# lan496/torch-m3gnet

Measured on AMD Instinct MI355X. Metric: atom-steps/sec (energy+forces) on 10k-atom PBC batch, 1/2/4/8 MI355X, higher is better.
Workload: dtype f32; 1 GPU; single 10000-atom fcc Cu PBC supercell per GPU (10x10x25 cells, a=3.61 A, jitter 0.025 A), r_cut 5 A / 3-body 4 A, default M3GNet (l_max=n_max=3, D=64, 3 blocks), energy+forces+stress; precision=fp32, atoms_per_gpu=10000, edges_per_gpu=420000, triplets_per_gpu=3060000

## Files before the change

torch-m3gnet_amd/csrc/m3g_api.hip:

```cpp
#include <cmath>
#include <cstdarg>
#include <cstdio>
#include <cstdlib>
#include <cstring>

#include "m3g_internal.h"

namespace m3g {

static thread_local char g_err[512] = "";
void set_error(const char* fmt, ...) {
  va_list ap;
  va_start(ap, fmt);
  vsnprintf(g_err, sizeof(g_err), fmt, ap);
  va_end(ap);
}

static inline size_t align_up(size_t x, size_t a = 256) { return (x + a - 1) / a * a; }

static void layout_mlp(MlpW& m, size_t& off) {
  auto take = [&](size_t n) { size_t r = off; off += (n + 63) / 64 * 64; return r; };
  m.w1a_t = take(kDP * 2 * kDP); m.w1b_t = take(kDP * 2 * kDP); m.w1c_t = take(kDP * 2 * kDP);
  m.b1 = take(2 * kDP);
  m.w2d_t = take(kDP * kDP); m.w2g_t = take(kDP * kDP);
// ... 312 lines not shown
    return M3G_OK;
  }
  if (strcmp(name, "save_p1") == 0) {
    plan->save_p1 = value != 0;
    return M3G_OK;
  }
  if (strcmp(name, "save_p2") == 0) {
    plan->save_p2 = value != 0;
    return M3G_OK;
  }
  if (strcmp(name, "rev_kernel") == 0) {
    if (value != 0 && value != 1) { set_error("rev_kernel must be 0 (node-MLP + edge-MLP kernel pair) or 1 (fused)"); return M3G_ERR_VALUE; }
    plan->rev_kernel = value;
    return M3G_OK;
  }
  if (strcmp(name, "small_tiles") == 0) {
    if (value < 0) { set_error("small_tiles must be >= 0"); return M3G_ERR_VALUE; }
    plan->small_tiles = value;
    plan->small_tiles_fwd = value;
    drop_graphs(plan);
    return M3G_OK;
  }
  if (strcmp(name, "small_tiles_fwd") == 0) {
    if (value < 0) { set_error("small_tiles_fwd must be >= 0"); return M3G_ERR_VALUE; }
    plan->small_tiles_fwd = value;
    drop_graphs(plan);
    return M3G_OK;
  }
  if (strcmp(name, "dp1_by_dst") == 0) {
    plan->dp1_by_dst = value != 0;
// ... 228 lines not shown
    M3G_HIP_CHECK(hipStreamWaitEvent(s, plan->ev_fork, 0));
  }
  auto join = [&]() -> int {
    if (via_side) {
      M3G_HIP_CHECK(hipEventRecord(plan->ev_join, s));
      M3G_HIP_CHECK(hipStreamWaitEvent(caller, plan->ev_join, 0));
    }
    return M3G_OK;
  };
  std::vector<unsigned char> key(sizeof(m3g_io) + sizeof(void*) * 2 + sizeof(size_t) + 4 * sizeof(int));
  unsigned char* k = key.data();
  memcpy(k, io, sizeof(m3g_io)); k += sizeof(m3g_io);
  memcpy(k, &workspace, sizeof(void*)); k += sizeof(void*);
  memcpy(k, &s, sizeof(void*)); k += sizeof(void*);
  memcpy(k, &workspace_bytes, sizeof(size_t)); k += sizeof(size_t);
  const int opts[4] = {plan->edge_kernel, plan->rev_kernel + 2 * plan->save_p1 + 4 * plan->save_p2 + 8 * plan->tb_moments + 16 * plan->precision + 64 * plan->readout_f16, plan->stress_mode, plan->overlap};
  memcpy(k, opts, sizeof(opts));
  for (auto& g : plan->graphs)
    if (g.key == key) { M3G_HIP_CHECK(hipGraphLaunch(g.exec, s)); return join(); }
  if (plan->graphs.size() >= 8) drop_graphs(plan);
  m3g_plan::GraphEntry ge;
  ge.key = key;
  M3G_HIP_CHECK(hipStreamBeginCapture(s, hipStreamCaptureModeThreadLocal));
  plan->capturing = true;
  const int rc = m3g_energy_forces(plan, io, workspace, workspace_bytes, (void*)s);
  plan->capturing = false;
  hipError_t e = hipStreamEndCapture(s, &ge.graph);
  if (rc != M3G_OK) { if (ge.graph) (void)hipGraphDestroy(ge.graph); return rc; }
  if (e != hipSuccess || !ge.graph) { set_error("hipStreamEndCapture failed: %s", hipGetErrorString(e)); return M3G_ERR_HIP; }
  e = hipGraphInstantiate(&ge.exec, ge.graph, nullptr, nullptr, 0);
  if (e != hipSuccess) { (void)hipGraphDestroy(ge.graph); set_error("hipGraphInstantiate failed: %s", hipGetErrorString(e)); return M3G_ERR_HIP; }
// ... 270 lines not shown
```

torch-m3gnet_amd/csrc/m3g_edge_common.h:

```cpp
#pragma once
#include <utility>

#include "m3g_device.h"
#include "m3g_internal.h"
#include "m3g_dual_chain.h"
#include "m3g_dual_f32.h"
#include "m3g_mfma_common.h"

namespace m3g {

constexpr int kFwdLdsFloats = 8 * kTbSteps * 64 + 2 * (8 * 4 * 4 * 64 + 2 * (4 * 4 * 4 * 64) + 2 * 4 * 64 + 4 * 64) + 4 * 64;
constexpr int kRevMlpFloats = 8 * 4 * 4 * 64 + 4 * (4 * 4 * 4 * 64) + 2 * 4 * 64 + 4 * 8 * 4 * 64 + 64 * 4;
constexpr int kRevEdgeFloats = kRevMlpFloats + 8 * kTbSteps * 64 + 8 * 4 * 64;
#ifndef M3G_WAVES_FWD
#define M3G_WAVES_FWD 16
#endif
constexpr int kWaves = M3G_WAVES_FWD;
#ifndef M3G_WAVES_FWD_H
#define M3G_WAVES_FWD_H 12
#endif
template <int PREC>
#ifndef M3G_WAVES_FWD_BF
#define M3G_WAVES_FWD_BF 12
#endif
// ... 397 lines not shown
  const float* e2_tile;
  float* de_soa;
  float* dcn;
  int de_is_zero;
  float* dm;
  float* dh;
  float* dp1;
  unsigned long long* stamps;
  float *seg_head, *seg_first;
  const float* p1;
  const float* p2;
  float w_inv;
  float* dp1_scale;
  const int32_t* in_pos;
  int split_tail;
};

__device__ __forceinline__ float sum_lane_quarters(float x) {
  const unsigned u = __builtin_bit_cast(unsigned, x);
  auto r16 = __builtin_amdgcn_permlane16_swap(u, u, false, false);
  const float y = __builtin_bit_cast(float, (unsigned)r16[0]) + __builtin_bit_cast(float, (unsigned)r16[1]);
  const unsigned v = __builtin_bit_cast(unsigned, y);
  auto r32 = __builtin_amdgcn_permlane32_swap(v, v, false, false);
  return __builtin_bit_cast(float, (unsigned)r32[0]) + __builtin_bit_cast(float, (unsigned)r32[1]);
}

__device__ __forceinline__ void store_dh(float* dh, int64_t edge, int64_t E, f32x4 dhv, int qd) {
  static_for<4>([&]<int rr>() { dhv[rr] = sum_lane_quarters(dhv[rr]); });
  if (qd == 0 && edge < E) *(f32x4*)(dh + edge * kRP) = dhv;
}
// ... 31 lines not shown
```

torch-m3gnet_amd/csrc/m3g_edge_rev_f32.hip:

```cpp
#include "m3g_edge_common.h"
#include "m3g_edge_split_rev.h"

namespace m3g {

MfmaRevF32Layout mfma_rev_f32_layout() {
  MfmaRevF32Layout L{};
  int off = 0;
  auto take = [&](int n) { int r = off; off += n; return r; };
  L.tb = take(8 * kTbSteps * 64);
  L.tbT = take(1 * 32 * 64);
  for (int m = 0; m < 2; ++m) {
    L.mlp[m].w2d = take(64 * 64);
    L.mlp[m].w2g = take(64 * 64);
    L.mlp[m].w1cT = take(4 * 32 * 64);
    L.mlp[m].b2 = take(2 * 4 * 64);
    L.mlp[m].wl = take(64 * 4);
    L.mlp[m].wld = take(4 * 64);
  }
  L.adj = take(4 * 64);
  L.adjp = take(64 * 4);
  L.total = off;
  return L;
}

constexpr int kRevF32Floats = 8 * kTbSteps * 64 + 32 * 64 + 2 * (2 * 64 * 64 + 4 * 32 * 64 + 2 * 4 * 64 + 64 * 4 + 4 * 64) + 4 * 64 + 64 * 4;
#ifndef M3G_WAVES_REV_F32
#define M3G_WAVES_REV_F32 8
#endif
constexpr int kWavesRevF32 = M3G_WAVES_REV_F32;

#ifndef M3G_NO_SCHED_FENCE
#define M3G_F32_FENCE() __builtin_amdgcn_sched_barrier(0)
#else
#define M3G_F32_FENCE() ((void)0)
#endif

template <bool NEED_DP1, int MLP, bool SAVED_P2>
__device__ __forceinline__ void mlp_reverse_f32(const float* lds, const MfmaMlpRevF32& L, const RevArgs& a, int64_t edge, int64_t drow, int64_t tile,
                                                int64_t ci, const SegMasks& sk, const f32x4& hv, const f32x4 (&d_upd)[4],
                                                f32x4 (&contrib)[4], f32x4& dhv, int lane, f32x4 (&d2)[8]) {
  const int qd = lane >> 4;
  f32x4 p1[SAVED_P2 ? 1 : 8];
  const float* p1_src = a.p1 + tile * (2 * kP1TileFloats) + MLP * kP1TileFloats + (threadIdx.x & 63) * 4;
  if constexpr (SAVED_P2) {
  } else {
    static_for<8>([&]<int ob>() { p1[ob] = load_tile4(p1_src + ob * 256); });
    bias_step<4, 0>(lds + L.b2, d2, lane);
    bias_step<4, 4>(lds + L.b2 + 4 * 64, d2, lane);
    static_for<2>([&]<int half>() {
      f32x4 hid[4];
      static_for<4>([&]<int ob>() {
        static_for<4>([&]<int r>() {
// ... 40 lines not shown
      const float d_out = du * s_lin, d_s = du * sd * sg;
      dhv[0] += d_s * w[0]; dhv[1] += d_s * w[1]; dhv[2] += d_s * w[2]; dhv[3] += d_s * w[3];
      d2[ob][r] = d_out * sg * (sgd * (1.f + p2d * (1.f - sgd)));
      d2[4 + ob][r] = d_out * sd * sg * (1.f - sg);
    });
#endif
    asm volatile("" : "+v"(dhv[0]), "+v"(dhv[1]), "+v"(dhv[2]), "+v"(dhv[3]));
  });
  zero(contrib);
  M3G_F32_FENCE();
  static_for<2>([&]<int half>() {
    f32x4 dp1[4];
    zero(dp1);
    f32x4 ds1[4];
    if constexpr (SAVED_P2) static_for<4>([&]<int ob>() { ds1[ob] = load_tile4(p1_src + (4 * half + ob) * 256); });
    chain_dual32_t<4, 4 * half, 0>(lds + (half == 0 ? L.w2d : L.w2g), d2, dp1, lane);
    if constexpr (SAVED_P2) static_for<4>([&]<int ob>() { dp1[ob] *= ds1[ob]; });
    else static_for<4>([&]<int ob>() { dp1[ob] *= p1[4 * half + ob]; });
    if (NEED_DP1 && edge < a.E) {
      float* row = a.dp1 + drow * (4 * kDP) + MLP * (2 * kDP) + half * kDP + 4 * qd;
      static_for<4>([&]<int ob>() { *(f32x4*)(row + ob * 16) = dp1[ob]; });
    }
    chain_f32<4, 4, 0, 0, 8, 4 * half>(lds + L.w1cT, dp1, contrib, lane);
    if (NEED_DP1) {
      if (edge >= a.E) zero(dp1);
      seg_scan(dp1, sk);
      seg_store<MLP * 8 + 4 * half>(dp1, sk, a.seg_head, a.seg_first, tile, ci, qd);
    }
    M3G_F32_FENCE();
  });
}

__device__ __forceinline__ void load_p2(const RevArgs& a, int64_t tile, int mlp, f32x4 (&d2)[8]) {
  const float* src = a.p2 + tile * (2 * kP1TileFloats) + mlp * kP1TileFloats + (threadIdx.x & 63) * 4;
  static_for<8>([&]<int ob>() { d2[ob] = load_tile4(src + ob * 256); });
}

template <int TBS, bool NEED_DP1, int WAVES, bool SAVED_P2>
__global__ void __launch_bounds__(64 * WAVES) k_edge_rev_f32(RevArgs a, MfmaRevF32Layout L) {
  __shared__ __attribute__((aligned(16))) float lds[kRevF32Floats + 4];
  int* q_head = reinterpret_cast<int*>(lds + kRevF32Floats);
  load_image(lds, a.img, kRevF32Floats, q_head);
  const int lane = threadIdx.x & 63, qd = lane >> 4;
  TileQueue queue(a.tiles, q_head);
  int tail = 0;
  if constexpr (SAVED_P2 && WAVES == 8) tail = (queue.count & 3) >= 1 && (queue.count & 3) <= a.split_tail ? (queue.count & 3) : 0;
  const int count_a = queue.count - tail;
  const int wave_id = __builtin_amdgcn_readfirstlane((int)(threadIdx.x >> 6));
  int ticket = queue.fetch(lane);
  int ci_i = 0, cj_i;
  if (ticket < count_a) load_ends(a.src, nullptr, queue.base + ticket, a.E, lane, ci_i, cj_i);
  constexpr bool FIRST = !NEED_DP1;
  while (ticket < count_a) {
    const int64_t tile = queue.base + ticket;
    ticket = queue.fetch(lane);
    const bool has_next = ticket < count_a;
    int nci = 0, ncj = 0;
    if (has_next) load_ends(a.src, nullptr, queue.base + ticket, a.E, lane, nci, ncj);
    int lv = lane;
    asm volatile("" : "+v"(lv));
    const int64_t edge = tile * kTileEdges + (lane & 15);
    const int64_t ec = edge < a.E ? edge : a.E - 1;
    const int64_t ci = ci_i;
// ... 20 lines not shown
    if (a.de_is_zero) {
      static_for<4>([&]<int blk>() { de[blk] = contrib[blk]; });
    } else {
      static_for<4>([&]<int blk>() { de[blk] = load_tile4(de_tile + blk * 256) + contrib[blk]; });
    }
    asm volatile("" : "+v"(lv));
    M3G_F32_FENCE();
#ifndef M3G_P2_PREFETCH
    if constexpr (SAVED_P2) load_p2(a, tile, 0, d2e);
#endif
    mlp_reverse_f32<NEED_DP1, 0, SAVED_P2>(lds, L.mlp[0], a, edge, drow, tile, ci, sk, hv, de, contrib, dhv, lv, d2e);
    static_for<4>([&]<int blk>() {
      de[blk] += contrib[blk];
      if (!FIRST) *(f32x4*)(de_tile + blk * 256) = de[blk];
    });
    if (FIRST) {
      const float hb = qd == 0 ? hv[0] : qd == 1 ? hv[1] : qd == 2 ? hv[2] : hv[3];
      static_for<4>([&]<int blk>() {
        const f32x4 pe = mfma16(lds[L.adj + blk * 64 + lv], hb, f32x4{0.f, 0.f, 0.f, 0.f});
        static_for<4>([&]<int r>() {
          const f32x4 w = *(const f32x4*)(lds + L.adjp + (blk * 16 + 4 * qd + r) * 4);
          const float t = de[blk][r] * fdsilu(pe[r]);
          dhv[0] += t * w[0]; dhv[1] += t * w[1]; dhv[2] += t * w[2]; dhv[3] += t * w[3];
        });
        asm volatile("" : "+v"(dhv[0]), "+v"(dhv[1]), "+v"(dhv[2]), "+v"(dhv[3]));
      });
    }
    f32x4 d8[8];
    tb_preact<TBS>(lds + L.tb, mb, d8, lv);
#ifndef M3G_F32_SCALAR_ACT
    static_for<4>([&]<int blk>() {
      static_for<2>([&]<int k>() {
        f32x2 sd, dsd;
        silu_pair(f32x2{d8[blk][2 * k], d8[blk][2 * k + 1]}, sd, dsd);
        const f32x2 sg = sigmoid_pair(f32x2{d8[4 + blk][2 * k], d8[4 + blk][2 * k + 1]});
        const f32x2 a_g = f32x2{de[blk][2 * k], de[blk][2 * k + 1]} * sg;
        const f32x2 dd = a_g * dsd, dgt = (a_g * sd) * (1.f - sg);
        d8[blk][2 * k] = dd[0]; d8[blk][2 * k + 1] = dd[1];
        d8[4 + blk][2 * k] = dgt[0]; d8[4 + blk][2 * k + 1] = dgt[1];
      });
    });
#else
    static_for<4>([&]<int blk>() {
      static_for<4>([&]<int r>() {
        const float p = d8[blk][r], sgd = fsigmoid(p), sg = fsigmoid(d8[4 + blk][r]);
        d8[blk][r] = de[blk][r] * sg * (sgd * (1.f + p * (1.f - sgd)));
        d8[4 + blk][r] = de[blk][r] * (p * sgd) * sg * (1.f - sg);
      });
    });
#endif
    f32x4 dmv[1];
    zero(dmv);
    chain_f32<1, 8>(lds + L.tbT, d8, dmv, lv);
    store_dh(a.dh, edge, a.E, dhv, qd);
    if (edge < a.E && arow >= 0) *(f32x4*)(a.dm + (int64_t)arow * kCP + 4 * qd) = dmv[0];
    ci_i = nci;
  }
  if constexpr (SAVED_P2 && WAVES == 8) {
    if (tail) {
      rev_split_run<TBS, NEED_DP1>(a, L, lds , lds, 2, wave_id >> 2, wave_id & 3, lane,
                                   queue.base + count_a + (wave_id >> 2), queue.base + queue.count, 2);
    }
  }
}

void launch_edge_rev_f32(const m3g_plan* plan, const Consts& c, const Topo& t, const Work& w, int b, const float* dx_new,
                         bool de_is_zero, hipStream_t s) {
  const int64_t tiles = tiles_for(t.E);
  if (tiles == 0) return;
  if (tiles <= plan->small_tiles && launch_edge_rev_split(plan, c, t, w, b, dx_new, de_is_zero, s)) return;
  const MfmaRevF32Layout L = mfma_rev_f32_layout();
  static_assert(kRevF32Floats * 4 + 16 <= 160 * 1024, "fused fp32 reverse image exceeds the LDS");
  const float* img = plan->d_mfma_revf32 + (size_t)b * L.total;
  RevArgs ar{t.E, tiles, img, t.src, t.dst, w.h, w.m[b], dx_new, t.act_id, nullptr, nullptr, nullptr, nullptr, w.de_soa, nullptr,
             de_is_zero ? 1 : 0, w.dm, w.dh_parts + (size_t)b * t.E * kRP, w.dp1, nullptr, w.seg_head, w.seg_first, w.p1_blk[b],
             saves_p2(plan) ? w.p2_blk[b] : nullptr, 1.f, nullptr, dp1_rows_by_dst(plan) ? t.in_pos : nullptr, plan->split_tail};
  static_assert(2 * kRevSplitGroupFloats + kRevSplitTabFloats <= kRevF32Floats, "the split tail's exchange buffers must fit in the image's LDS");
  constexpr int WV = kWavesRevF32;
  dim3 grid(grid_for_tiles(tiles, WV)), block(64 * WV);
  const bool p2 = saves_p2(plan);
#define M3G_REV_F32_LAUNCH(NEED, P2) M3G_TBS_SWITCH(c.C, hipLaunchKernelGGL((k_edge_rev_f32<TBS, NEED, WV, P2>), grid, block, 0, s, ar, L))
  if (b > 0) { if (p2) { M3G_REV_F32_LAUNCH(true, true); } else { M3G_REV_F32_LAUNCH(true, false); } }
  else { if (p2) { M3G_REV_F32_LAUNCH(false, true); } else { M3G_REV_F32_LAUNCH(false, false); } }
#undef M3G_REV_F32_LAUNCH
}

}
```

torch-m3gnet_amd/csrc/m3g_internal.h:

```cpp
#pragma once
#include <hip/hip_runtime.h>

#include <cstddef>
#include <cstdint>
#include <map>
#include <string>
#include <vector>

#include "../../include/m3gnet_hip.h"

namespace m3g {

constexpr int kDP = 64;
constexpr int kLCap = 4;
constexpr int kRCap = 4;
constexpr int kCP = 16;
constexpr int kRP = 4;
constexpr int kMaxBlocks = 8;
constexpr int kPrecF32 = 0;
constexpr int kPrecBf16x3 = 1;
constexpr int kPrecF16x3 = 2;
constexpr int kNumPrec = 3;

void set_error(const char* fmt, ...);
// ... 104 lines not shown
  int w2d, w2g;
  int w1cT;
  int b2;
  int wl;
  int wld;
};
struct MfmaRevF32Layout {
  int tb;
  int tbT;
  MfmaMlpRevF32 mlp[2];
  int adj;
  int adjp;
  int total;
};
MfmaRevF32Layout mfma_rev_f32_layout();
constexpr int kNodeRowBlocks = 33;
constexpr int kNodeImgFloats = kNodeRowBlocks * 16 * 64 + kNodeRowBlocks * 16;
struct ReadoutImg {
  static constexpr int w1 = 0;
  static constexpr int w2d = w1 + 8 * 2 * 512;
  static constexpr int w2g = w2d + 4 * 2 * 512;
  static constexpr int w2dT = w2g + 4 * 2 * 512;
  static constexpr int w2gT = w2dT + 4 * 2 * 512;
  static constexpr int w1T = w2gT + 4 * 2 * 512;
  static constexpr int b1 = w1T + 4 * 4 * 512;
  static constexpr int b2 = b1 + 128;
  static constexpr int w3 = b2 + 128;
  static constexpr int b3 = w3 + 128;
  static constexpr int total = b3 + 4;
};
// ... 3 lines not shown

}

struct m3g_plan {
  m3g_config cfg;
  m3g::Consts consts;
  m3g::WeightLayout wl;
  std::map<std::string, std::vector<float>> params;
  std::map<std::string, std::vector<float>> cvals;
  float* d_weights = nullptr;
  float* d_mfma_fwd[m3g::kNumPrec] = {nullptr, nullptr, nullptr};
  float* d_mfma_rev[m3g::kNumPrec] = {nullptr, nullptr, nullptr};
  float* d_mfma_revf = nullptr;
  float* d_mfma_revf_h = nullptr;
  float* d_mfma_revf32 = nullptr;
  float* d_node_img[m3g::kNumPrec] = {nullptr, nullptr, nullptr};
  int precision = m3g::kPrecF32;
  float w_scale_inv = 1.f;
  int save_p1 = 1;
  int save_p2 = 1;
  int device = -1;
  bool generic = false;
  float* d_generic = nullptr;
  std::map<std::string, size_t> generic_off;
  float* d_readout_img = nullptr;
  float* d_readout_img_h = nullptr;
  float ro_w_scale_inv = 1.f;
  int small_tiles_fwd = 3072;
  int small_tiles = 1536;
  int dp1_by_dst = 0;
  int split_node_tiles = 128;
  int fuse_node_tb = 1;
  int debug_node_tb_polls = 0;
  int split_tail = 1;
  int small_launches = 1;
  int rev_kernel = 1;
  bool readout_f16 = false;
  bool legendre_ref = false;
  bool tb_moments = true;
  int stress_mode = 0;
  int edge_kernel = 1;
  int stamp_target = 0;
  unsigned long long* d_stamps = nullptr;
  bool committed = false;
  bool debug_force_move = false;
  mutable hipStream_t side_stream = nullptr;
  mutable hipEvent_t ev_fork = nullptr, ev_join = nullptr;
  int overlap = 0;
  int graph_replay = 0;
  struct GraphEntry { std::vector<unsigned char> key; hipGraph_t graph = nullptr; hipGraphExec_t exec = nullptr; };
  mutable std::vector<GraphEntry> graphs;
// ... 207 lines not shown
```

torch-m3gnet_amd/csrc/m3g_pack_mfma.hip:

```cpp
#include <cmath>
#include <cstring>

#include "m3g_dual_chain.h"
#include "m3g_dual_f32.h"
#include "m3g_internal.h"

namespace m3g {

MfmaFwdLayout mfma_fwd_layout() {
  MfmaFwdLayout L{};
  int off = 0;
  auto take = [&](int n) { int r = off; off += n; return r; };
  L.tb = take(8 * kTbSteps * 64);
  for (int m = 0; m < 2; ++m) {
    L.mlp[m].w1c = take(8 * 4 * 4 * 64);
    L.mlp[m].w2d = take(4 * 4 * 4 * 64);
    L.mlp[m].w2g = take(4 * 4 * 4 * 64);
    L.mlp[m].b2 = take(2 * 4 * 64);
    L.mlp[m].wl = take(4 * 1 * 64);
  }
  L.adj = take(4 * 64);
  L.total = off;
  return L;
}
// ... 125 lines not shown
}

template <class F>
static void chain_image_p(int prec, float wscale, float* img, int OB, int KS, F get) {
  if (prec == kPrecBf16x3) chain_image(img, OB, KS, get);
  else if (prec == kPrecF16x3) chain_image_h(img, OB, KS, wscale, get);
  else f32_chain_image(img, OB, 8 * KS, get);
}

void free_mfma_images(m3g_plan* plan) {
  auto drop = [](float*& p) { if (p) { (void)hipFree(p); p = nullptr; } };
  for (int prec = 0; prec < kNumPrec; ++prec) { drop(plan->d_mfma_fwd[prec]); drop(plan->d_mfma_rev[prec]); drop(plan->d_node_img[prec]); }
  drop(plan->d_mfma_revf);
  drop(plan->d_mfma_revf_h);
  drop(plan->d_mfma_revf32);
  drop(plan->d_readout_img);
  drop(plan->d_readout_img_h);
}

static int upload(float*& dst, const std::vector<float>& host) {
  if (!dst) M3G_HIP_CHECK(hipMalloc((void**)&dst, host.size() * sizeof(float)));
  M3G_HIP_CHECK(hipMemcpy(dst, host.data(), host.size() * sizeof(float), hipMemcpyHostToDevice));
  return M3G_OK;
}

int pack_mfma_images(m3g_plan* plan) {
  const m3g_config& cfg = plan->cfg;
  const int D = cfg.embedding_dim, R = cfg.n_max, C = cfg.l_max * cfg.n_max, B = cfg.num_blocks;
  const MfmaFwdLayout F = mfma_fwd_layout();
  const MfmaRevLayout Rv = mfma_rev_layout();
  const MfmaRevFusedLayout Rf = mfma_rev_fused_layout();
  const MfmaRevF32Layout R32 = mfma_rev_f32_layout();
  std::vector<float> revf((size_t)std::max(B, 1) * Rf.total, 0.f), revf32((size_t)std::max(B, 1) * R32.total, 0.f);
  std::vector<float> revfh((size_t)std::max(B, 1) * Rf.total, 0.f);
  float wscale = 1.f;
  {
    float wmax = 0.f;
    for (const auto& kv : plan->params) {
      const std::string& k = kv.first;
      const bool chain_weight = k.find(".concat_") != std::string::npos || k.find(".gated_mlp.") != std::string::npos ||
                                k.find(".linear_sigmoid1.weight") != std::string::npos;
      if (!chain_weight || k.find(".bias") != std::string::npos) continue;
      for (float v : kv.second) wmax = std::max(wmax, std::fabs(v));
    }
    int e = 0;
    if (wmax > 0.f && std::isfinite(wmax)) (void)std::frexp(wmax, &e);
    wscale = std::ldexp(1.f, 13 - e);
// ... 19 lines not shown
    float* rf = revf.data() + (size_t)b * Rf.total;
    float* rfh = revfh.data() + (size_t)b * Rf.total;
    direct_image(rf + Rf.tb, 8, kTbSteps, tbw);
    tb_image_h(rfh + Rf.tb, wscale, tbw);
    auto tbT = [&](int row, int k) -> float {
      const float* w = k < 64 ? wd : wg;
      int o = k & 63;
      return (row < C && o < D) ? w[(size_t)o * C + row] : 0.f;
    };
    chain_image_p(prec, wscale, r + Rv.tbT, 1, 4, tbT);
    chain_image(rf + Rf.tbT, 1, 4, tbT);
    chain_image_h(rfh + Rf.tbT, 1, 4, wscale, tbT);
    float* r32 = revf32.data() + (size_t)b * R32.total;
    direct_image(r32 + R32.tb, 8, kTbSteps, tbw);
    f32_chain_image(r32 + R32.tbT, 1, 32, tbT);
    {
      const float* wadj = plan->params.at("model.5.linear.weight").data();
      auto adj = [&](int row, int k) -> float { return (row < D && k < R) ? wadj[(size_t)row * R + k] : 0.f; };
      direct_image(f + F.adj, 4, 1, adj);
      direct_image(rf + Rf.adj, 4, 1, adj);
      direct_image(rfh + Rf.adj, 4, 1, adj);
      direct_image(r32 + R32.adj, 4, 1, adj);
      for (int o = 0; o < 64; ++o)
        for (int rr = 0; rr < 4; ++rr) rf[Rf.adjp + o * 4 + rr] = rfh[Rf.adjp + o * 4 + rr] = r32[R32.adjp + o * 4 + rr] = adj(o, rr);
    }
    {
      float* ni = node.data() + (size_t)b * kNodeImgFloats;
      const char* names[2] = {".concat_edge_update", ".concat_node_update"};
      const float* w1[2][2];
      const float* b1[2][2];
      for (int m = 0; m < 2; ++m) {
        w1[m][0] = plan->params.at(cv + names[m] + ".dense.0.weight").data();
        w1[m][1] = plan->params.at(cv + names[m] + ".gate.0.weight").data();
        b1[m][0] = plan->params.at(cv + names[m] + ".dense.0.bias").data();
        b1[m][1] = plan->params.at(cv + names[m] + ".gate.0.bias").data();
      }
      const float* ws = plan->params.at(tb + ".linear_sigmoid1.weight").data();
      const float* bs = plan->params.at(tb + ".linear_sigmoid1.bias").data();
      auto row_w = [&](int row, int k) -> float {
// ... 62 lines not shown
      bias_image(rf + Rf.mlp[m].b2);
      memcpy(rf + Rf.mlp[m].wl, rm + Rv.mlp.wl, sizeof(float) * 64 * 4);
      direct_image(rf + Rf.mlp[m].wld, 4, 1, [&](int row, int k) -> float { return (row < D && k < R) ? wl[(size_t)row * R + k] : 0.f; });
      pack_dual_image_h(rfh + Rf.mlp[m].w1c, 128, wscale, w1c);
      pack_dual_image_h(rfh + Rf.mlp[m].w2d, 64, wscale, sq(w2d));
      pack_dual_image_h(rfh + Rf.mlp[m].w2g, 64, wscale, sq(w2g));
      bias_image(rfh + Rf.mlp[m].b2);
      memcpy(rfh + Rf.mlp[m].wl, rm + Rv.mlp.wl, sizeof(float) * 64 * 4);
      memcpy(rfh + Rf.mlp[m].wld, rf + Rf.mlp[m].wld, sizeof(float) * 4 * 64);
      pack_dual32_image(r32 + R32.mlp[m].w2d, 64, sq(w2d));
      pack_dual32_image(r32 + R32.mlp[m].w2g, 64, sq(w2g));
      f32_chain_image(r32 + R32.mlp[m].w1cT, 4, 32, [&](int row, int k) -> float { return w1c(k, row); });
      bias_image(r32 + R32.mlp[m].b2);
      memcpy(r32 + R32.mlp[m].wl, rm + Rv.mlp.wl, sizeof(float) * 64 * 4);
      memcpy(r32 + R32.mlp[m].wld, rf + Rf.mlp[m].wld, sizeof(float) * 4 * 64);
    }
  }
  { int rc = upload(plan->d_mfma_fwd[prec], fwd); if (rc) return rc; }
  { int rc = upload(plan->d_mfma_rev[prec], rev); if (rc) return rc; }
  { int rc = upload(plan->d_node_img[prec], node); if (rc) return rc; }
  }
  {
    const std::string ro = "model." + std::to_string(6 + 2 * B) + ".gated.";
    const float* w1d = plan->params.at(ro + "dense.0.weight").data();
    const float* w1g = plan->params.at(ro + "gate.0.weight").data();
    const float* w2d = plan->params.at(ro + "dense.2.weight").data();
    const float* w2g = plan->params.at(ro + "gate.2.weight").data();
    std::vector<float> img(ReadoutImg::total, 0.f);
    auto sq = [&](const float* w) { return [=](int row, int k) -> float { return (row < D && k < D) ? w[(size_t)row * D + k] : 0.f; }; };
    auto sqT = [&](const float* w) { return [=](int row, int k) -> float { return (row < D && k < D) ? w[(size_t)k * D + row] : 0.f; }; };
// ... 24 lines not shown
    if (wmax > 0.f) (void)std::frexp(wmax, &e);
    const float ro_scale = std::ldexp(1.f, 13 - e);
    plan->ro_w_scale_inv = std::ldexp(1.f, e - 13);
    std::vector<float> imh(img);
    chain_image_h(imh.data() + ReadoutImg::w1, 8, 2, ro_scale, w1);
    chain_image_h(imh.data() + ReadoutImg::w2d, 4, 2, ro_scale, sq(w2d));
    chain_image_h(imh.data() + ReadoutImg::w2g, 4, 2, ro_scale, sq(w2g));
    chain_image_h(imh.data() + ReadoutImg::w2dT, 4, 2, ro_scale, sqT(w2d));
    chain_image_h(imh.data() + ReadoutImg::w2gT, 4, 2, ro_scale, sqT(w2g));
    chain_image_h(imh.data() + ReadoutImg::w1T, 4, 4, ro_scale, [&](int row, int k) -> float { return w1(k, row); });
    { int rc = upload(plan->d_readout_img_h, imh); if (rc) return rc; }
  }
  { int rc = upload(plan->d_mfma_revf, revf); if (rc) return rc; }
  { int rc = upload(plan->d_mfma_revf_h, revfh); if (rc) return rc; }
  { int rc = upload(plan->d_mfma_revf32, revf32); if (rc) return rc; }
  return M3G_OK;
}

}
```

Before: 4.280 million atom-steps/s.

## Use three-part bf16 split MFMA products in fp32 reverse edge kernel

Adds a reverse-pass path, on by default, that runs the fp32 MLP reverse chains as bf16 MFMAs on three-way split (hi/mid/lo) weights and gradients. The aim is to reach near-fp32 accuracy with faster bf16 matrix instructions. Because the split weight images are larger, the kernel now runs in two phases, first the node MLP and then the edge MLP plus three-body embedding, reloading LDS in between. The split costs eight MFMAs per step plus extra conversion work, a second pass over tiles with an extra dh read-modify-write, and a __syncthreads barrier between the phases.

New measurement: 4.252 million atom-steps/s, median of 6. About the same (-0.7%).

```diff
diff --git a/torch-m3gnet_amd/csrc/m3g_api.hip b/torch-m3gnet_amd/csrc/m3g_api.hip
--- a/torch-m3gnet_amd/csrc/m3g_api.hip
+++ b/torch-m3gnet_amd/csrc/m3g_api.hip
@@ -350,6 +350,12 @@
     plan->rev_kernel = value;
     return M3G_OK;
   }
+  if (strcmp(name, "rev_arith") == 0) {
+    if (value != 0 && value != 1) { set_error("rev_arith must be 0 (fp32 MFMA chains) or 1 (exact three-part bf16 products)"); return M3G_ERR_VALUE; }
+    plan->rev_arith = value;
+    drop_graphs(plan);
+    return M3G_OK;
+  }
   if (strcmp(name, "small_tiles") == 0) {
     if (value < 0) { set_error("small_tiles must be >= 0"); return M3G_ERR_VALUE; }
     plan->small_tiles = value;
@@ -608,7 +614,7 @@
   memcpy(k, &workspace, sizeof(void*)); k += sizeof(void*);
   memcpy(k, &s, sizeof(void*)); k += sizeof(void*);
   memcpy(k, &workspace_bytes, sizeof(size_t)); k += sizeof(size_t);
-  const int opts[4] = {plan->edge_kernel, plan->rev_kernel + 2 * plan->save_p1 + 4 * plan->save_p2 + 8 * plan->tb_moments + 16 * plan->precision + 64 * plan->readout_f16, plan->stress_mode, plan->overlap};
+  const int opts[4] = {plan->edge_kernel, plan->rev_kernel + 2 * plan->save_p1 + 4 * plan->save_p2 + 8 * plan->tb_moments + 16 * plan->precision + 64 * plan->readout_f16 + 128 * plan->rev_arith, plan->stress_mode, plan->overlap};
   memcpy(k, opts, sizeof(opts));
   for (auto& g : plan->graphs)
     if (g.key == key) { M3G_HIP_CHECK(hipGraphLaunch(g.exec, s)); return join(); }
diff --git a/torch-m3gnet_amd/csrc/m3g_edge_common.h b/torch-m3gnet_amd/csrc/m3g_edge_common.h
--- a/torch-m3gnet_amd/csrc/m3g_edge_common.h
+++ b/torch-m3gnet_amd/csrc/m3g_edge_common.h
@@ -435,6 +435,7 @@
   float* dp1_scale;
   const int32_t* in_pos;
   int split_tail;
+  const float* img3 = nullptr;
 };
 
 __device__ __forceinline__ float sum_lane_quarters(float x) {
diff --git a/torch-m3gnet_amd/csrc/m3g_edge_rev_f32.hip b/torch-m3gnet_amd/csrc/m3g_edge_rev_f32.hip
--- a/torch-m3gnet_amd/csrc/m3g_edge_rev_f32.hip
+++ b/torch-m3gnet_amd/csrc/m3g_edge_rev_f32.hip
@@ -1,5 +1,6 @@
 #include "m3g_edge_common.h"
 #include "m3g_edge_split_rev.h"
+#include "m3g_tri_chain.h"
 
 namespace m3g {
 
@@ -35,7 +36,7 @@
 #define M3G_F32_FENCE() ((void)0)
 #endif
 
-template <bool NEED_DP1, int MLP, bool SAVED_P2>
+template <bool NEED_DP1, int MLP, bool SAVED_P2, bool TRI = false>
 __device__ __forceinline__ void mlp_reverse_f32(const float* lds, const MfmaMlpRevF32& L, const RevArgs& a, int64_t edge, int64_t drow, int64_t tile,
                                                 int64_t ci, const SegMasks& sk, const f32x4& hv, const f32x4 (&d_upd)[4],
                                                 f32x4 (&contrib)[4], f32x4& dhv, int lane, f32x4 (&d2)[8]) {
@@ -106,14 +107,16 @@
     zero(dp1);
     f32x4 ds1[4];
     if constexpr (SAVED_P2) static_for<4>([&]<int ob>() { ds1[ob] = load_tile4(p1_src + (4 * half + ob) * 256); });
-    chain_dual32_t<4, 4 * half, 0>(lds + (half == 0 ? L.w2d : L.w2g), d2, dp1, lane);
+    if constexpr (TRI) chain3_t<2, 64, 4 * half>(lds + (half == 0 ? L.w2d : L.w2g), d2, dp1, lane);
+    else chain_dual32_t<4, 4 * half, 0>(lds + (half == 0 ? L.w2d : L.w2g), d2, dp1, lane);
     if constexpr (SAVED_P2) static_for<4>([&]<int ob>() { dp1[ob] *= ds1[ob]; });
     else static_for<4>([&]<int ob>() { dp1[ob] *= p1[4 * half + ob]; });
     if (NEED_DP1 && edge < a.E) {
       float* row = a.dp1 + drow * (4 * kDP) + MLP * (2 * kDP) + half * kDP + 4 * qd;
       static_for<4>([&]<int ob>() { *(f32x4*)(row + ob * 16) = dp1[ob]; });
     }
-    chain_f32<4, 4, 0, 0, 8, 4 * half>(lds + L.w1cT, dp1, contrib, lane);
+    if constexpr (TRI) chain3_t<2, 128, 0, 0, 4 * half>(lds + L.w1cT, dp1, contrib, lane);
+    else chain_f32<4, 4, 0, 0, 8, 4 * half>(lds + L.w1cT, dp1, contrib, lane);
     if (NEED_DP1) {
       if (edge >= a.E) zero(dp1);
       seg_scan(dp1, sk);
@@ -123,22 +126,148 @@
   });
 }
 
+template <int TBS, bool FIRST>
+__device__ __forceinline__ f32x4 tb_embed_reverse(const float* lds, int tb, int tbT, int adj, int adjp, const f32x4 (&de)[4], const f32x4& hv,
+                                                  const float (&mb)[TBS], f32x4& dhv, int lv) {
+  const int qd = (threadIdx.x & 63) >> 4;
+  if (FIRST) {
+    const float hb = qd == 0 ? hv[0] : qd == 1 ? hv[1] : qd == 2 ? hv[2] : hv[3];
+    static_for<4>([&]<int blk>() {
+      const f32x4 pe = mfma16(lds[adj + blk * 64 + lv], hb, f32x4{0.f, 0.f, 0.f, 0.f});
+      static_for<4>([&]<int r>() {
+        const f32x4 w = *(const f32x4*)(lds + adjp + (blk * 16 + 4 * qd + r) * 4);
+        const float t = de[blk][r] * fdsilu(pe[r]);
+        dhv[0] += t * w[0]; dhv[1] += t * w[1]; dhv[2] += t * w[2]; dhv[3] += t * w[3];
+      });
+      asm volatile("" : "+v"(dhv[0]), "+v"(dhv[1]), "+v"(dhv[2]), "+v"(dhv[3]));
+    });
+  }
+  f32x4 d8[8];
+  tb_preact<TBS>(lds + tb, mb, d8, lv);
+#ifndef M3G_F32_SCALAR_ACT
+  static_for<4>([&]<int blk>() {
+    static_for<2>([&]<int k>() {
+      f32x2 sd, dsd;
+      silu_pair(f32x2{d8[blk][2 * k], d8[blk][2 * k + 1]}, sd, dsd);
+      const f32x2 sg = sigmoid_pair(f32x2{d8[4 + blk][2 * k], d8[4 + blk][2 * k + 1]});
+      const f32x2 a_g = f32x2{de[blk][2 * k], de[blk][2 * k + 1]} * sg;
+      const f32x2 dd = a_g * dsd, dgt = (a_g * sd) * (1.f - sg);
+      d8[blk][2 * k] = dd[0]; d8[blk][2 * k + 1] = dd[1];
+      d8[4 + blk][2 * k] = dgt[0]; d8[4 + blk][2 * k + 1] = dgt[1];
+    });
+  });
+#else
+  static_for<4>([&]<int blk>() {
+    static_for<4>([&]<int r>() {
+      const float p = d8[blk][r], sgd = fsigmoid(p), sg = fsigmoid(d8[4 + blk][r]);
+      d8[blk][r] = de[blk][r] * sg * (sgd * (1.f + p * (1.f - sgd)));
+      d8[4 + blk][r] = de[blk][r] * (p * sgd) * sg * (1.f - sg);
+    });
+  });
+#endif
+  f32x4 dmv[1];
+  zero(dmv);
+  chain_f32<1, 8>(lds + tbT, d8, dmv, lv);
+  return dmv[0];
+}
+
 __device__ __forceinline__ void load_p2(const RevArgs& a, int64_t tile, int mlp, f32x4 (&d2)[8]) {
   const float* src = a.p2 + tile * (2 * kP1TileFloats) + mlp * kP1TileFloats + (threadIdx.x & 63) * 4;
   static_for<8>([&]<int ob>() { d2[ob] = load_tile4(src + ob * 256); });
 }
 
-template <int TBS, bool NEED_DP1, int WAVES, bool SAVED_P2>
-__global__ void __launch_bounds__(64 * WAVES) k_edge_rev_f32(RevArgs a, MfmaRevF32Layout L) {
+__device__ __forceinline__ void store_dh_add(float* dh, int64_t edge, int64_t E, f32x4 dhv, int qd) {
+  static_for<4>([&]<int rr>() { dhv[rr] = sum_lane_quarters(dhv[rr]); });
+  if (qd == 0 && edge < E) *(f32x4*)(dh + edge * kRP) = *(const f32x4*)(dh + edge * kRP) + dhv;
+}
+
+template <int TBS, bool NEED_DP1>
+__device__ __forceinline__ void rev3_phases(const RevArgs& a, const MfmaRev3Layout& L3, float* lds, int* q_head, const TileQueue& queue,
+                                            int count_a, int lane) {
+  const int qd = lane >> 4;
+  constexpr bool FIRST = !NEED_DP1;
+  int ticket = queue.fetch(lane);
+  int ci_i = 0, cj_i;
+  if (ticket < count_a) load_ends(a.src, nullptr, queue.base + ticket, a.E, lane, ci_i, cj_i);
+  while (ticket < count_a) {
+    const int64_t tile = queue.base + ticket;
+    ticket = queue.fetch(lane);
+    int nci = 0, ncj = 0;
+    if (ticket < count_a) load_ends(a.src, nullptr, queue.base + ticket, a.E, lane, nci, ncj);
+    int lv = lane;
+    asm volatile("" : "+v"(lv));
+    const int64_t edge = tile * kTileEdges + (lane & 15);
+    const int64_t ec = edge < a.E ? edge : a.E - 1;
+    const int64_t ci = ci_i;
+    const int64_t drow = (NEED_DP1 && a.in_pos) ? (int64_t)a.in_pos[ec] : edge;
+    const SegMasks sk = seg_masks((int)ci, lane);
+    float* de_tile = a.de_soa + tile * kTileFloats + lane * 4;
+    const f32x4 hv = *(const f32x4*)(a.h + ec * kRP);
+    f32x4 dhv = {0.f, 0.f, 0.f, 0.f};
+    f32x4 dmsg[4], contrib[4], d2n[8];
+    const float* xrow = a.dx_new + ci * kDP + 4 * qd;
+    static_for<4>([&]<int blk>() { dmsg[blk] = *(const f32x4*)(xrow + blk * 16); });
+    load_p2(a, tile, 1, d2n);
+    mlp_reverse_f32<NEED_DP1, 1, true, true>(lds, L3.node, a, edge, drow, tile, ci, sk, hv, dmsg, contrib, dhv, lv, d2n);
+    if (!a.de_is_zero) static_for<4>([&]<int blk>() { contrib[blk] = load_tile4(de_tile + blk * 256) + contrib[blk]; });
+    static_for<4>([&]<int blk>() { *(f32x4*)(de_tile + blk * 256) = contrib[blk]; });
+    store_dh(a.dh, edge, a.E, dhv, qd);
+    ci_i = nci;
+  }
+  __syncthreads();
+  load_image(lds, a.img3 + L3.a_total, L3.b_total, q_head);
+  ticket = queue.fetch(lane);
+  ci_i = 0;
+  if (ticket < count_a) load_ends(a.src, nullptr, queue.base + ticket, a.E, lane, ci_i, cj_i);
+  while (ticket < count_a) {
+    const int64_t tile = queue.base + ticket;
+    ticket = queue.fetch(lane);
+    int nci = 0, ncj = 0;
+    if (ticket < count_a) load_ends(a.src, nullptr, queue.base + ticket, a.E, lane, nci, ncj);
+    int lv = lane;
+    asm volatile("" : "+v"(lv));
+    const int64_t edge = tile * kTileEdges + (lane & 15);
+    const int64_t ec = edge < a.E ? edge : a.E - 1;
+    const int64_t ci = ci_i;
+    const int64_t drow = (NEED_DP1 && a.in_pos) ? (int64_t)a.in_pos[ec] : edge;
+    const SegMasks sk = seg_masks((int)ci, lane);
+    float* de_tile = a.de_soa + tile * kTileFloats + lane * 4;
+    const f32x4 hv = *(const f32x4*)(a.h + ec * kRP);
+    f32x4 dhv = {0.f, 0.f, 0.f, 0.f};
+    float mb[TBS];
+    const int arow = a.act_id[ec];
+    static_for<TBS>([&]<int s>() { mb[s] = arow >= 0 ? a.m[(int64_t)arow * kCP + 4 * s + qd] : 0.f; });
+    f32x4 de[4], contrib[4], d2e[8];
+    static_for<4>([&]<int blk>() { de[blk] = load_tile4(de_tile + blk * 256); });
+    load_p2(a, tile, 0, d2e);
+    mlp_reverse_f32<NEED_DP1, 0, true, true>(lds, L3.edge, a, edge, drow, tile, ci, sk, hv, de, contrib, dhv, lv, d2e);
+    static_for<4>([&]<int blk>() {
+      de[blk] += contrib[blk];
+      if (!FIRST) *(f32x4*)(de_tile + blk * 256) = de[blk];
+    });
+    const f32x4 dmv = tb_embed_reverse<TBS, FIRST>(lds, L3.tb, L3.tbT, L3.adj, L3.adjp, de, hv, mb, dhv, lv);
+    store_dh_add(a.dh, edge, a.E, dhv, qd);
+    if (edge < a.E && arow >= 0) *(f32x4*)(a.dm + (int64_t)arow * kCP + 4 * qd) = dmv;
+    ci_i = nci;
+  }
+}
+
+template <int TBS, bool NEED_DP1, int WAVES, bool SAVED_P2, bool TRI = false>
+__global__ void __launch_bounds__(64 * WAVES) k_edge_rev_f32(RevArgs a, MfmaRevF32Layout L, MfmaRev3Layout L3) {
+  static_assert(!TRI || SAVED_P2, "the three-part arithmetic runs on the saved layer-2 pre-activations");
   __shared__ __attribute__((aligned(16))) float lds[kRevF32Floats + 4];
   int* q_head = reinterpret_cast<int*>(lds + kRevF32Floats);
-  load_image(lds, a.img, kRevF32Floats, q_head);
+  if constexpr (TRI) load_image(lds, a.img3, L3.a_total, q_head);
+  else load_image(lds, a.img, kRevF32Floats, q_head);
   const int lane = threadIdx.x & 63, qd = lane >> 4;
   TileQueue queue(a.tiles, q_head);
   int tail = 0;
   if constexpr (SAVED_P2 && WAVES == 8) tail = (queue.count & 3) >= 1 && (queue.count & 3) <= a.split_tail ? (queue.count & 3) : 0;
   const int count_a = queue.count - tail;
   const int wave_id = __builtin_amdgcn_readfirstlane((int)(threadIdx.x >> 6));
+  if constexpr (TRI) {
+    rev3_phases<TBS, NEED_DP1>(a, L3, lds, q_head, queue, count_a, lane);
+  } else {
   int ticket = queue.fetch(lane);
   int ci_i = 0, cj_i;
   if (ticket < count_a) load_ends(a.src, nullptr, queue.base + ticket, a.E, lane, ci_i, cj_i);
@@ -189,52 +318,16 @@
       de[blk] += contrib[blk];
       if (!FIRST) *(f32x4*)(de_tile + blk * 256) = de[blk];
     });
-    if (FIRST) {
-      const float hb = qd == 0 ? hv[0] : qd == 1 ? hv[1] : qd == 2 ? hv[2] : hv[3];
-      static_for<4>([&]<int blk>() {
-        const f32x4 pe = mfma16(lds[L.adj + blk * 64 + lv], hb, f32x4{0.f, 0.f, 0.f, 0.f});
-        static_for<4>([&]<int r>() {
-          const f32x4 w = *(const f32x4*)(lds + L.adjp + (blk * 16 + 4 * qd + r) * 4);
-          const float t = de[blk][r] * fdsilu(pe[r]);
-          dhv[0] += t * w[0]; dhv[1] += t * w[1]; dhv[2] += t * w[2]; dhv[3] += t * w[3];
-        });
-        asm volatile("" : "+v"(dhv[0]), "+v"(dhv[1]), "+v"(dhv[2]), "+v"(dhv[3]));
-      });
-    }
-    f32x4 d8[8];
-    tb_preact<TBS>(lds + L.tb, mb, d8, lv);
-#ifndef M3G_F32_SCALAR_ACT
-    static_for<4>([&]<int blk>() {
-      static_for<2>([&]<int k>() {
-        f32x2 sd, dsd;
-        silu_pair(f32x2{d8[blk][2 * k], d8[blk][2 * k + 1]}, sd, dsd);
-        const f32x2 sg = sigmoid_pair(f32x2{d8[4 + blk][2 * k], d8[4 + blk][2 * k + 1]});
-        const f32x2 a_g = f32x2{de[blk][2 * k], de[blk][2 * k + 1]} * sg;
-        const f32x2 dd = a_g * dsd, dgt = (a_g * sd) * (1.f - sg);
-        d8[blk][2 * k] = dd[0]; d8[blk][2 * k + 1] = dd[1];
-        d8[4 + blk][2 * k] = dgt[0]; d8[4 + blk][2 * k + 1] = dgt[1];
-      });
-    });
-#else
-    static_for<4>([&]<int blk>() {
-      static_for<4>([&]<int r>() {
-        const float p = d8[blk][r], sgd = fsigmoid(p), sg = fsigmoid(d8[4 + blk][r]);
-        d8[blk][r] = de[blk][r] * sg * (sgd * (1.f + p * (1.f - sgd)));
-        d8[4 + blk][r] = de[blk][r] * (p * sgd) * sg * (1.f - sg);
-      });
-    });
-#endif
-    f32x4 dmv[1];
-    zero(dmv);
-    chain_f32<1, 8>(lds + L.tbT, d8, dmv, lv);
+    const f32x4 dmv = tb_embed_reverse<TBS, FIRST>(lds, L.tb, L.tbT, L.adj, L.adjp, de, hv, mb, dhv, lv);
     store_dh(a.dh, edge, a.E, dhv, qd);
-    if (edge < a.E && arow >= 0) *(f32x4*)(a.dm + (int64_t)arow * kCP + 4 * qd) = dmv[0];
+    if (edge < a.E && arow >= 0) *(f32x4*)(a.dm + (int64_t)arow * kCP + 4 * qd) = dmv;
     ci_i = nci;
+  }
   }
   if constexpr (SAVED_P2 && WAVES == 8) {
     if (tail) {
-      rev_split_run<TBS, NEED_DP1>(a, L, lds , lds, 2, wave_id >> 2, wave_id & 3, lane,
-                                   queue.base + count_a + (wave_id >> 2), queue.base + queue.count, 2);
+      rev_split_run<TBS, NEED_DP1>(a, L, TRI ? a.img : lds , lds, 2, wave_id >> 2,
+                                   wave_id & 3, lane, queue.base + count_a + (wave_id >> 2), queue.base + queue.count, 2);
     }
   }
 }
@@ -254,9 +347,14 @@
   constexpr int WV = kWavesRevF32;
   dim3 grid(grid_for_tiles(tiles, WV)), block(64 * WV);
   const bool p2 = saves_p2(plan);
-#define M3G_REV_F32_LAUNCH(NEED, P2) M3G_TBS_SWITCH(c.C, hipLaunchKernelGGL((k_edge_rev_f32<TBS, NEED, WV, P2>), grid, block, 0, s, ar, L))
-  if (b > 0) { if (p2) { M3G_REV_F32_LAUNCH(true, true); } else { M3G_REV_F32_LAUNCH(true, false); } }
-  else { if (p2) { M3G_REV_F32_LAUNCH(false, true); } else { M3G_REV_F32_LAUNCH(false, false); } }
+  constexpr MfmaRev3Layout L3 = mfma_rev3_layout();
+  static_assert(mfma_rev3_layout().a_total <= kRevF32Floats && mfma_rev3_layout().b_total <= kRevF32Floats, "a phase image exceeds the kernel's LDS");
+  const bool tri = p2 && plan->rev_arith == 1;
+  if (tri) ar.img3 = plan->d_mfma_rev3 + (size_t)b * (L3.a_total + L3.b_total);
+#define M3G_REV_F32_LAUNCH(NEED, P2, TRI) \
+  M3G_TBS_SWITCH(c.C, hipLaunchKernelGGL((k_edge_rev_f32<TBS, NEED, WV, P2, TRI>), grid, block, 0, s, ar, L, L3))
+  if (b > 0) { if (tri) { M3G_REV_F32_LAUNCH(true, true, true); } else if (p2) { M3G_REV_F32_LAUNCH(true, true, false); } else { M3G_REV_F32_LAUNCH(true, false, false); } }
+  else { if (tri) { M3G_REV_F32_LAUNCH(false, true, true); } else if (p2) { M3G_REV_F32_LAUNCH(false, true, false); } else { M3G_REV_F32_LAUNCH(false, false, false); } }
 #undef M3G_REV_F32_LAUNCH
 }
 
diff --git a/torch-m3gnet_amd/csrc/m3g_internal.h b/torch-m3gnet_amd/csrc/m3g_internal.h
--- a/torch-m3gnet_amd/csrc/m3g_internal.h
+++ b/torch-m3gnet_amd/csrc/m3g_internal.h
@@ -142,6 +142,36 @@
   int total;
 };
 MfmaRevF32Layout mfma_rev_f32_layout();
+struct MfmaRev3Layout {
+  MfmaMlpRevF32 node;
+  int a_total;
+  MfmaMlpRevF32 edge;
+  int tb, tbT, adj, adjp;
+  int b_total;
+};
+constexpr MfmaRev3Layout mfma_rev3_layout() {
+  MfmaRev3Layout L{};
+  int off = 0;
+  auto take = [&](int n) { int r = off; off += n; return r; };
+  auto mlp = [&](MfmaMlpRevF32& M) {
+    M.w2d = take(64 * 96);
+    M.w2g = take(64 * 96);
+    M.w1cT = take(128 * 96);
+    M.b2 = take(2 * 4 * 64);
+    M.wl = take(64 * 4);
+    M.wld = take(4 * 64);
+  };
+  mlp(L.node);
+  L.a_total = off;
+  off = 0;
+  mlp(L.edge);
+  L.tb = take(8 * kTbSteps * 64);
+  L.tbT = take(1 * 32 * 64);
+  L.adj = take(4 * 64);
+  L.adjp = take(64 * 4);
+  L.b_total = off;
+  return L;
+}
 constexpr int kNodeRowBlocks = 33;
 constexpr int kNodeImgFloats = kNodeRowBlocks * 16 * 64 + kNodeRowBlocks * 16;
 struct ReadoutImg {
@@ -175,6 +205,7 @@
   float* d_mfma_revf = nullptr;
   float* d_mfma_revf_h = nullptr;
   float* d_mfma_revf32 = nullptr;
+  float* d_mfma_rev3 = nullptr;
   float* d_node_img[m3g::kNumPrec] = {nullptr, nullptr, nullptr};
   int precision = m3g::kPrecF32;
   float w_scale_inv = 1.f;
@@ -196,6 +227,7 @@
   int split_tail = 1;
   int small_launches = 1;
   int rev_kernel = 1;
+  int rev_arith = 1;
   bool readout_f16 = false;
   bool legendre_ref = false;
   bool tb_moments = true;
diff --git a/torch-m3gnet_amd/csrc/m3g_pack_mfma.hip b/torch-m3gnet_amd/csrc/m3g_pack_mfma.hip
--- a/torch-m3gnet_amd/csrc/m3g_pack_mfma.hip
+++ b/torch-m3gnet_amd/csrc/m3g_pack_mfma.hip
@@ -4,6 +4,7 @@
 #include "m3g_dual_chain.h"
 #include "m3g_dual_f32.h"
 #include "m3g_internal.h"
+#include "m3g_tri_chain.h"
 
 namespace m3g {
 
@@ -163,6 +164,7 @@
   drop(plan->d_mfma_revf);
   drop(plan->d_mfma_revf_h);
   drop(plan->d_mfma_revf32);
+  drop(plan->d_mfma_rev3);
   drop(plan->d_readout_img);
   drop(plan->d_readout_img_h);
 }
@@ -180,6 +182,9 @@
   const MfmaRevLayout Rv = mfma_rev_layout();
   const MfmaRevFusedLayout Rf = mfma_rev_fused_layout();
   const MfmaRevF32Layout R32 = mfma_rev_f32_layout();
+  constexpr MfmaRev3Layout R3 = mfma_rev3_layout();
+  constexpr int kR3 = R3.a_total + R3.b_total;
+  std::vector<float> rev3((size_t)std::max(B, 1) * kR3, 0.f);
   std::vector<float> revf((size_t)std::max(B, 1) * Rf.total, 0.f), revf32((size_t)std::max(B, 1) * R32.total, 0.f);
   std::vector<float> revfh((size_t)std::max(B, 1) * Rf.total, 0.f);
   float wscale = 1.f;
@@ -229,6 +234,10 @@
     float* r32 = revf32.data() + (size_t)b * R32.total;
     direct_image(r32 + R32.tb, 8, kTbSteps, tbw);
     f32_chain_image(r32 + R32.tbT, 1, 32, tbT);
+    float* r3a = rev3.data() + (size_t)b * kR3;
+    float* r3b = r3a + R3.a_total;
+    direct_image(r3b + R3.tb, 8, kTbSteps, tbw);
+    f32_chain_image(r3b + R3.tbT, 1, 32, tbT);
     {
       const float* wadj = plan->params.at("model.5.linear.weight").data();
       auto adj = [&](int row, int k) -> float { return (row < D && k < R) ? wadj[(size_t)row * R + k] : 0.f; };
@@ -236,8 +245,10 @@
       direct_image(rf + Rf.adj, 4, 1, adj);
       direct_image(rfh + Rf.adj, 4, 1, adj);
       direct_image(r32 + R32.adj, 4, 1, adj);
+      direct_image(r3b + R3.adj, 4, 1, adj);
       for (int o = 0; o < 64; ++o)
-        for (int rr = 0; rr < 4; ++rr) rf[Rf.adjp + o * 4 + rr] = rfh[Rf.adjp + o * 4 + rr] = r32[R32.adjp + o * 4 + rr] = adj(o, rr);
+        for (int rr = 0; rr < 4; ++rr)
+          rf[Rf.adjp + o * 4 + rr] = rfh[Rf.adjp + o * 4 + rr] = r32[R32.adjp + o * 4 + rr] = r3b[R3.adjp + o * 4 + rr] = adj(o, rr);
     }
     {
       float* ni = node.data() + (size_t)b * kNodeImgFloats;
@@ -330,6 +341,14 @@
       bias_image(r32 + R32.mlp[m].b2);
       memcpy(r32 + R32.mlp[m].wl, rm + Rv.mlp.wl, sizeof(float) * 64 * 4);
       memcpy(r32 + R32.mlp[m].wld, rf + Rf.mlp[m].wld, sizeof(float) * 4 * 64);
+      float* r3 = m == 1 ? r3a : r3b;
+      const MfmaMlpRevF32& M3 = m == 1 ? R3.node : R3.edge;
+      pack_dual_image3(r3 + M3.w2d, 64, sq(w2d));
+      pack_dual_image3(r3 + M3.w2g, 64, sq(w2g));
+      pack_dual_image3(r3 + M3.w1cT, 128, w1c);
+      memcpy(r3 + M3.b2, r32 + R32.mlp[m].b2, sizeof(float) * 2 * 4 * 64);
+      memcpy(r3 + M3.wl, r32 + R32.mlp[m].wl, sizeof(float) * 64 * 4);
+      memcpy(r3 + M3.wld, r32 + R32.mlp[m].wld, sizeof(float) * 4 * 64);
     }
   }
   { int rc = upload(plan->d_mfma_fwd[prec], fwd); if (rc) return rc; }
@@ -384,6 +403,7 @@
   { int rc = upload(plan->d_mfma_revf, revf); if (rc) return rc; }
   { int rc = upload(plan->d_mfma_revf_h, revfh); if (rc) return rc; }
   { int rc = upload(plan->d_mfma_revf32, revf32); if (rc) return rc; }
+  { int rc = upload(plan->d_mfma_rev3, rev3); if (rc) return rc; }
   return M3G_OK;
 }
 
diff --git a/torch-m3gnet_amd/csrc/m3g_tri_chain.h b/torch-m3gnet_amd/csrc/m3g_tri_chain.h
--- /dev/null
+++ b/torch-m3gnet_amd/csrc/m3g_tri_chain.h
@@ -0,0 +1,86 @@
+#pragma once
+#include "m3g_dual_chain.h"
+
+namespace m3g {
+
+__device__ __forceinline__ void split8_3(const f32x4& a, const f32x4& b, bf16x8& hi, bf16x8& mid, bf16x8& lo) {
+  static_for<8>([&]<int j>() {
+    const float x = j < 4 ? a[j & 3] : b[j & 3];
+    const __bf16 h = (__bf16)x;
+    const float r = x - (float)h;
+    const __bf16 m = (__bf16)r;
+    hi[j] = h;
+    mid[j] = m;
+    lo[j] = (__bf16)(r - (float)m);
+  });
+}
+
+template <int KS, int ROWS, int DOFF = 0, int AOFF = 0, int KB0 = 0, int ND, int NA>
+__device__ __forceinline__ void chain3_t(const float* img, const f32x4 (&d)[ND], f32x4 (&acc)[NA], int lane) {
+  static_assert(DOFF + 2 * KS <= ND && AOFF + 4 <= NA && (KB0 + 2 * KS) * 16 <= ROWS, "chain3_t operand out of range");
+  const int q = lane >> 4, qp = (lane & 15) >> 2, p = lane & 3;
+  const int row_lo = 4 * q + qp, sw = dual_swz(row_lo);
+  const char* base = reinterpret_cast<const char*>(img) + (row_lo >> 3) * 1024 + (row_lo & 7) * 64;
+  constexpr int plane = 512, part = ROWS * 128;
+  M3G_CHAIN_PRIO(1);
+  static_for<KS>([&]<int s>() {
+    constexpr int r0 = (KB0 + 2 * s) * 2048, r1 = (KB0 + 2 * s + 1) * 2048;
+    auto fetch = [&]<int P>(bf16x8 (&dst)[4]) {
+      static_for<4>([&]<int ob>() {
+        const char* u = base + P * part + (ob & 1) * plane + ((((ob >> 1) * 4 + p) ^ sw) << 3);
+        dst[ob] = join_halves(__builtin_amdgcn_ds_read_tr16_b64_v4i16((lds_s16x4_ptr)(u + r0)),
+                              __builtin_amdgcn_ds_read_tr16_b64_v4i16((lds_s16x4_ptr)(u + r1)));
+      });
+    };
+    bf16x8 ah[4], am[4], al[4];
+    fetch.template operator()<2>(al);
+    fetch.template operator()<1>(am);
+    fetch.template operator()<0>(ah);
+    bf16x8 bh, bm, bl;
+    split8_3(d[DOFF + 2 * s], d[DOFF + 2 * s + 1], bh, bm, bl);
+    static_for<4>([&]<int ob>() { acc[AOFF + ob] = mfma_bf16(al[ob], bm, acc[AOFF + ob]); });
+    static_for<4>([&]<int ob>() { acc[AOFF + ob] = mfma_bf16(am[ob], bl, acc[AOFF + ob]); });
+    static_for<4>([&]<int ob>() { acc[AOFF + ob] = mfma_bf16(am[ob], bm, acc[AOFF + ob]); });
+    static_for<4>([&]<int ob>() { acc[AOFF + ob] = mfma_bf16(al[ob], bh, acc[AOFF + ob]); });
+    static_for<4>([&]<int ob>() { acc[AOFF + ob] = mfma_bf16(ah[ob], bl, acc[AOFF + ob]); });
+    static_for<4>([&]<int ob>() { acc[AOFF + ob] = mfma_bf16(am[ob], bh, acc[AOFF + ob]); });
+    static_for<4>([&]<int ob>() { acc[AOFF + ob] = mfma_bf16(ah[ob], bm, acc[AOFF + ob]); });
+    static_for<4>([&]<int ob>() { acc[AOFF + ob] = mfma_bf16(ah[ob], bh, acc[AOFF + ob]); });
+  });
+  M3G_CHAIN_PRIO(0);
+}
+
+inline uint16_t bf16_rn_host(float w) {
+  uint32_t u;
+  memcpy(&u, &w, 4);
+  if ((u & 0x7F800000u) == 0x7F800000u) return (uint16_t)(u >> 16);
+  const uint32_t r = u + 0x7FFFu + ((u >> 16) & 1u);
+  if ((r & 0x7F800000u) == 0x7F800000u) return (uint16_t)(u >> 16);
+  return (uint16_t)(r >> 16);
+}
+inline float bf16_to_float_host(uint16_t h) {
+  const uint32_t u = (uint32_t)h << 16;
+  float f;
+  memcpy(&f, &u, 4);
+  return f;
+}
+template <class F>
+inline void pack_dual_image3(float* img, int rows, F get) {
+  uint16_t* hi = reinterpret_cast<uint16_t*>(img);
+  uint16_t* mid = hi + (size_t)rows * 64;
+  uint16_t* lo = mid + (size_t)rows * 64;
+  for (int row = 0; row < rows; ++row)
+    for (int col = 0; col < 64; ++col) {
+      const float w = get(row, col);
+      const uint16_t h = bf16_rn_host(w);
+      const float r = w - bf16_to_float_host(h);
+      const uint16_t m = bf16_rn_host(r);
+      const size_t idx = (size_t)(dual_unit_byte(rows, row, col >> 2) >> 1) + (col & 3);
+      hi[idx] = h;
+      mid[idx] = m;
+      lo[idx] = bf16_rn_host(r - bf16_to_float_host(m));
+    }
+}
+inline size_t dual_image3_floats(int rows) { return (size_t)rows * 96; }
+
+}
```
